# Zhongxu-Wang/ArtSpeech

Hardware: AMD Instinct MI355X
Metric: mel frames/sec (whole job; per-GPU = value / n_gpus), acoustic-model inference path, batch 32 x 200-frame utterances (higher is better)
Workload: dtype f32 (f16x3 split-operand MFMA, fp32 accumulate)

## Files before the change

### artspeech_amd/csrc/lstm.hip

```cpp
#include "common.h"
#include "artspeech_hip.h"
#define AS_FILE_CLS AS_CLS_LSTM

#define NB 2

static __device__ __forceinline__ float sigmoidf_(float x) { return __builtin_amdgcn_rcpf(1.0f + __expf(-x)); }
static __device__ __forceinline__ float tanhf_(float x)
{
    const float e = __expf(-2.0f * fabsf(x));
    const float t = (1.0f - e) * __builtin_amdgcn_rcpf(1.0f + e);
    return x < 0.f ? -t : t;
}

template <int CTRL>
static __device__ __forceinline__ float quad_dpp(float v)
{
    return __int_as_float(__builtin_amdgcn_mov_dpp(__float_as_int(v), CTRL, 0xf, 0xf, true));
}

struct LstmJobs { BiLstmJob j[AS_MAX_LSTM_JOBS]; };

static __device__ __forceinline__ void lds_barrier()
{
    asm volatile("s_waitcnt lgkmcnt(0)\n\ts_barrier" ::: "memory");
}

template <int HREG>
__global__ void __launch_bounds__(HREG ? 4 * HREG : 1024)
bilstm_kernel(const LstmJobs jobs, const int* __restrict__ col_off, int B, int Hrt)
{
    extern __shared__ __attribute__((aligned(16))) float sm[];
    const int H = HREG ? HREG : Hrt;
    float* hs = sm;
    float* gs = sm + 2 * H * NB;
    __shared__ int s_off[NB], s_len[NB];

    const BiLstmJob job = jobs.j[blockIdx.z];
    const int dir = blockIdx.y;
    const int u0 = blockIdx.x * NB;
    const int r = threadIdx.x;
    const int G = 4 * H;
    if (r < NB) {
        const int u = u0 + r;
        s_off[r] = u < B ? col_off[u] : 0;
        s_len[r] = u < B ? col_off[u + 1] - col_off[u] : 0;
    }
    for (int i = r; i < 2 * H * NB; i += G) hs[i] = 0.f;
    __syncthreads();
    int Lmax = 0;
#pragma unroll
    for (int u = 0; u < NB; ++u) Lmax = s_len[u] > Lmax ? s_len[u] : Lmax;

    const float* w = job.whh_t + (size_t)dir * H * G + r;
    float wreg[HREG ? HREG : 1];
    if (HREG) {
#pragma unroll
        for (int k = 0; k < HREG; ++k) wreg[k] = w[(size_t)k * G];
    }
    const int unit = r % H, q = r / H;
    float c = 0.f;

    auto load_gx = [&](int t, float (&g)[NB]) {
#pragma unroll
        for (int u = 0; u < NB; ++u) {
            const int L = s_len[u];
            const int pos = dir ? L - 1 - t : t;
            g[u] = (t < L) ? job.gx_tm[(size_t)(s_off[u] + pos) * job.ldg + dir * G + r] : 0.f;
        }
    };
    float gnext[NB];
    load_gx(0, gnext);

    for (int t = 0; t < Lmax; ++t) {
        const float* hc = hs + (t & 1) * H * NB;
        float* hn = hs + ((t + 1) & 1) * H * NB;
        float acc[NB];
#pragma unroll
        for (int u = 0; u < NB; ++u) acc[u] = gnext[u];
        if (t + 1 < Lmax) load_gx(t + 1, gnext);
        if (HREG) {
#pragma unroll
            for (int k = 0; k < HREG; ++k) {
                const float2 h2 = *reinterpret_cast<const float2*>(hc + k * NB);
                acc[0] += wreg[k] * h2.x; acc[1] += wreg[k] * h2.y;
            }
        } else {
            for (int k0 = 0; k0 < H; k0 += 8) {
                float wk[8];
#pragma unroll
                for (int i = 0; i < 8; ++i) wk[i] = w[(size_t)(k0 + i) * G];
#pragma unroll
                for (int i = 0; i < 8; ++i) {
                    const float2 h2 = *reinterpret_cast<const float2*>(hc + (k0 + i) * NB);
                    acc[0] += wk[i] * h2.x; acc[1] += wk[i] * h2.y;
                }
            }
        }
        *reinterpret_cast<float2*>(gs + r * NB) = make_float2(acc[0], acc[1]);
        lds_barrier();
        if (q < NB) {
            const int u = q;
            const int L = s_len[u];
            if (t < L) {
                const float ig = sigmoidf_(gs[(unit)*NB + u]);
                const float fg = sigmoidf_(gs[(H + unit) * NB + u]);
                const float gg = tanhf_(gs[(2 * H + unit) * NB + u]);
                const float og = sigmoidf_(gs[(3 * H + unit) * NB + u]);
                c = fg * c + ig * gg;
                const float hv = og * tanhf_(c);
                hn[unit * NB + u] = hv;
                const int pos = dir ? L - 1 - t : t;
                job.out[(size_t)(dir * H + unit) * job.ldo + s_off[u] + pos] = hv;
            }
        }
        lds_barrier();
    }
}

template <int H, int KREG, int KLDS>
__global__ void __launch_bounds__(2 * H)
bilstm_big_kernel(const LstmJobs jobs, const int* __restrict__ col_off, int B)
{
    constexpr int G = 4 * H, NT = 2 * H, KS = H - KREG - KLDS, SB = 4;
    static_assert(KS >= 0 && KS % SB == 0, "split of the k range");
    extern __shared__ __attribute__((aligned(16))) float sm[];
    float* hs = sm;
    float* gs = hs + 2 * H * NB;
    float* wl = gs + G * NB;
    __shared__ int s_off[NB], s_len[NB];

    const BiLstmJob job = jobs.j[blockIdx.z];
    const int dir = blockIdx.y;
    const int u0 = blockIdx.x * NB;
    const int tid = threadIdx.x;
    if (tid < NB) {
        const int u = u0 + tid;
        s_off[tid] = u < B ? col_off[u] : 0;
        s_len[tid] = u < B ? col_off[u + 1] - col_off[u] : 0;
    }
    for (int i = tid; i < 2 * H * NB; i += NT) hs[i] = 0.f;
    const float* w = job.whh_t + (size_t)dir * H * G + tid;
    float wa[KREG], wb[KREG];
#pragma unroll
    for (int k = 0; k < KREG; ++k) {
        wa[k] = w[(size_t)k * G];
        wb[k] = w[(size_t)k * G + NT];
    }
#pragma unroll 4
    for (int k = 0; k < KLDS; ++k) {
        wl[k * G + tid] = w[(size_t)(KREG + k) * G];
        wl[k * G + NT + tid] = w[(size_t)(KREG + k) * G + NT];
    }
    const float* ws = w + (size_t)(KREG + KLDS) * G;
    __syncthreads();
    int Lmax = 0;
#pragma unroll
    for (int u = 0; u < NB; ++u) Lmax = s_len[u] > Lmax ? s_len[u] : Lmax;
    const int unit = tid % H, q = tid / H;
    float c = 0.f;

    auto load_gx = [&](int t, float (&ga)[NB], float (&gb)[NB]) {
#pragma unroll
        for (int u = 0; u < NB; ++u) {
            const int L = s_len[u];
            const int pos = dir ? L - 1 - t : t;
            const float* p = job.gx_tm + (size_t)(s_off[u] + pos) * job.ldg + dir * G + tid;
            ga[u] = (t < L) ? p[0] : 0.f;
            gb[u] = (t < L) ? p[NT] : 0.f;
        }
    };
    float gna[NB], gnb[NB];
    load_gx(0, gna, gnb);

    for (int t = 0; t < Lmax; ++t) {
        asm volatile("" ::: "memory");
        const float* hc = hs + (t & 1) * H * NB;
        float* hn = hs + ((t + 1) & 1) * H * NB;
        float a0 = gna[0], a1 = gna[1], b0 = gnb[0], b1 = gnb[1];
        if (t + 1 < Lmax) load_gx(t + 1, gna, gnb);
        float ka[SB], kb[SB];
#pragma unroll
        for (int i = 0; i < SB; ++i) {
            ka[i] = ws[(size_t)i * G];
            kb[i] = ws[(size_t)i * G + NT];
        }
#pragma unroll
        for (int k = 0; k < KREG; ++k) {
            const float2 h2 = *reinterpret_cast<const float2*>(hc + k * NB);
            a0 += wa[k] * h2.x; a1 += wa[k] * h2.y;
            b0 += wb[k] * h2.x; b1 += wb[k] * h2.y;
            if ((k & 7) == 7) asm volatile("" ::: "memory");
        }
#pragma unroll 4
        for (int k = 0; k < KLDS; ++k) {
            const float va = wl[k * G + tid], vb = wl[k * G + NT + tid];
            const float2 h2 = *reinterpret_cast<const float2*>(hc + (KREG + k) * NB);
            a0 += va * h2.x; a1 += va * h2.y;
            b0 += vb * h2.x; b1 += vb * h2.y;
        }
        for (int k0 = 0; k0 < KS; k0 += SB) {
            float na[SB], nb[SB];
            const int kn = k0 + SB < KS ? k0 + SB : k0;
#pragma unroll
            for (int i = 0; i < SB; ++i) {
                na[i] = ws[(size_t)(kn + i) * G];
                nb[i] = ws[(size_t)(kn + i) * G + NT];
            }
#pragma unroll
            for (int i = 0; i < SB; ++i) {
                const float2 h2 = *reinterpret_cast<const float2*>(hc + (KREG + KLDS + k0 + i) * NB);
                a0 += ka[i] * h2.x; a1 += ka[i] * h2.y;
                b0 += kb[i] * h2.x; b1 += kb[i] * h2.y;
            }
#pragma unroll
            for (int i = 0; i < SB; ++i) { ka[i] = na[i]; kb[i] = nb[i]; }
        }
        *reinterpret_cast<float2*>(gs + tid * NB) = make_float2(a0, a1);
        *reinterpret_cast<float2*>(gs + (NT + tid) * NB) = make_float2(b0, b1);
        lds_barrier();
        {
            const int u = q;
            const int L = s_len[u];
            if (t < L) {
                const float ig = sigmoidf_(gs[(unit)*NB + u]);
                const float fg = sigmoidf_(gs[(H + unit) * NB + u]);
                const float gg = tanhf_(gs[(2 * H + unit) * NB + u]);
                const float og = sigmoidf_(gs[(3 * H + unit) * NB + u]);
                c = fg * c + ig * gg;
                const float hv = og * tanhf_(c);
                hn[unit * NB + u] = hv;
                const int pos = dir ? L - 1 - t : t;
                job.out[(size_t)(dir * H + unit) * job.ldo + s_off[u] + pos] = hv;
            }
        }
        lds_barrier();
    }
}

template <int H>
__global__ void __launch_bounds__(4 * H)
bilstm_quad_kernel(const LstmJobs jobs, const int* __restrict__ col_off, int B)
{
    constexpr int KQ = H / 4, G = 4 * H;
    __shared__ __attribute__((aligned(16))) float hs[2][H][NB];
    __shared__ int s_off[NB], s_len[NB];
    const BiLstmJob job = jobs.j[blockIdx.z];
    const int dir = blockIdx.y, u0 = blockIdx.x * NB;
    const int tid = threadIdx.x, unit = tid >> 2, kq = tid & 3;
    if (tid < NB) {
        const int u = u0 + tid;
        s_off[tid] = u < B ? col_off[u] : 0;
        s_len[tid] = u < B ? col_off[u + 1] - col_off[u] : 0;
    }
    for (int i = tid; i < 2 * H * NB; i += G) (&hs[0][0][0])[i] = 0.f;
    __syncthreads();
    const int L0 = s_len[0], L1 = s_len[1], o0 = s_off[0], o1 = s_off[1];
    const int Lmax = L0 > L1 ? L0 : L1;

    float w[4][KQ];
    const float* wp = job.whh_t + (size_t)dir * H * G + unit;
#pragma unroll
    for (int g = 0; g < 4; ++g)
#pragma unroll
        for (int kk = 0; kk < KQ; ++kk) w[g][kk] = wp[(size_t)(kq * KQ + kk) * G + g * H];

    const float* gxp = job.gx_tm + dir * G + kq * H + unit;
    auto load_gx = [&](int t, float& g0, float& g1) {
        g0 = (t < L0) ? gxp[(size_t)(o0 + (dir ? L0 - 1 - t : t)) * job.ldg] : 0.f;
        g1 = (t < L1) ? gxp[(size_t)(o1 + (dir ? L1 - 1 - t : t)) * job.ldg] : 0.f;
    };
    constexpr int PF = 4;
    float gq0[PF], gq1[PF];
#pragma unroll
    for (int j = 0; j < PF; ++j) load_gx(j, gq0[j], gq1[j]);
    float c = 0.f;
    const int my_u = kq & 1, my_L = my_u ? L1 : L0, my_o = my_u ? o1 : o0;

    for (int t0 = 0; t0 < Lmax; t0 += PF) {
#pragma unroll
      for (int j = 0; j < PF; ++j) {
        const int t = t0 + j;
        if (t >= Lmax) break;
        const float(*hc)[NB] = hs[t & 1];
        float(*hn)[NB] = hs[(t + 1) & 1];
        float acc[4][2];
#pragma unroll
        for (int g = 0; g < 4; ++g) {
            acc[g][0] = (g == kq) ? gq0[j] : 0.f;
            acc[g][1] = (g == kq) ? gq1[j] : 0.f;
        }
        load_gx(t + PF, gq0[j], gq1[j]);
#pragma unroll
        for (int kk = 0; kk < KQ; ++kk) {
            const float2 h2 = *reinterpret_cast<const float2*>(&hc[kq * KQ + kk][0]);
#pragma unroll
            for (int g = 0; g < 4; ++g) {
                acc[g][0] += w[g][kk] * h2.x;
                acc[g][1] += w[g][kk] * h2.y;
            }
        }
        float pre[4];
#pragma unroll
        for (int g = 0; g < 4; ++g) {
            float a0 = acc[g][0], a1 = acc[g][1];
            a0 += __shfl_xor(a0, 1); a1 += __shfl_xor(a1, 1);
            a0 += __shfl_xor(a0, 2); a1 += __shfl_xor(a1, 2);
            pre[g] = my_u ? a1 : a0;
        }
        if (kq < 2 && t < my_L) {
            const float ig = sigmoidf_(pre[0]), fg = sigmoidf_(pre[1]), gg = tanhf_(pre[2]), og = sigmoidf_(pre[3]);
            c = fg * c + ig * gg;
            const float hv = og * tanhf_(c);
            hn[unit][my_u] = hv;
            job.out[(size_t)(dir * H + unit) * job.ldo + my_o + (dir ? my_L - 1 - t : t)] = hv;
        }
        lds_barrier();
      }
    }
}

typedef float lf2 __attribute__((ext_vector_type(2)));
template <int H>
__global__ void __launch_bounds__(4 * H)
bilstm_quad1_kernel(const LstmJobs jobs, const int* __restrict__ col_off, int B)
{
    constexpr int KQ = H / 4, G = 4 * H;
    static_assert(KQ % 4 == 0, "quarter of the hidden vector in float4 steps");
    __shared__ __attribute__((aligned(16))) float hs[2][H];
    const BiLstmJob job = jobs.j[blockIdx.z];
    const int dir = blockIdx.y, u = blockIdx.x;
    const int tid = threadIdx.x, unit = tid >> 2, kq = tid & 3;
    const int o0 = col_off[u], L = col_off[u + 1] - o0;
    if (L <= 0) return;
    for (int i = tid; i < 2 * H; i += G) (&hs[0][0])[i] = 0.f;
    __syncthreads();

    lf2 wif[KQ], wgo[KQ];
    const float* wp = job.whh_t + (size_t)dir * H * G + unit;
#pragma unroll
    for (int kk = 0; kk < KQ; ++kk) {
        const float* r = wp + (size_t)(kq * KQ + kk) * G;
        wif[kk] = lf2{r[0], r[H]};
        wgo[kk] = lf2{r[2 * H], r[3 * H]};
    }
    const float* gxp = job.gx_tm + dir * G + kq * H + unit;
    auto load_gx = [&](int t) { return (t < L) ? gxp[(size_t)(o0 + (dir ? L - 1 - t : t)) * job.ldg] : 0.f; };
    constexpr int PF = 4;
    float gq[PF];
#pragma unroll
    for (int j = 0; j < PF; ++j) gq[j] = load_gx(j);
    float c = 0.f;
    float* outp = job.out + (size_t)(dir * H + unit) * job.ldo + o0;

    for (int t0 = 0; t0 < L; t0 += PF) {
#pragma unroll
        for (int j = 0; j < PF; ++j) {
            const int t = t0 + j;
            if (t >= L) break;
            const float* hc = hs[t & 1] + kq * KQ;
            float* hn = hs[(t + 1) & 1];
            const float gx = gq[j];
            gq[j] = load_gx(t + PF);
            lf2 aif0 = {0.f, 0.f}, ago0 = {0.f, 0.f}, aif1 = {0.f, 0.f}, ago1 = {0.f, 0.f};
#pragma unroll
            for (int k4 = 0; k4 < KQ; k4 += 4) {
                const float4 h4 = *reinterpret_cast<const float4*>(hc + k4);
                aif0 += wif[k4] * lf2{h4.x, h4.x};
                ago0 += wgo[k4] * lf2{h4.x, h4.x};
                aif1 += wif[k4 + 1] * lf2{h4.y, h4.y};
                ago1 += wgo[k4 + 1] * lf2{h4.y, h4.y};
                aif0 += wif[k4 + 2] * lf2{h4.z, h4.z};
                ago0 += wgo[k4 + 2] * lf2{h4.z, h4.z};
                aif1 += wif[k4 + 3] * lf2{h4.w, h4.w};
                ago1 += wgo[k4 + 3] * lf2{h4.w, h4.w};
            }
            float pre[4] = {aif0[0] + aif1[0], aif0[1] + aif1[1], ago0[0] + ago1[0], ago0[1] + ago1[1]};
#pragma unroll
            for (int g = 0; g < 4; ++g) {
                pre[g] += quad_dpp<0xB1>(pre[g]);
                pre[g] += quad_dpp<0x4E>(pre[g]);
            }
            const float sc = kq == 2 ? 2.f : 1.f;
            const float x = (kq == 0 ? pre[0] : kq == 1 ? pre[1] : kq == 2 ? pre[2] : pre[3]) + gx;
            const float act = fmaf(__builtin_amdgcn_rcpf(1.0f + __expf(-sc * x)), sc, 1.0f - sc);
            const float ig = quad_dpp<0x00>(act), fg = quad_dpp<0x55>(act), gg = quad_dpp<0xAA>(act), og = quad_dpp<0xFF>(act);
            c = fg * c + ig * gg;
            const float hv = og * fmaf(__builtin_amdgcn_rcpf(1.0f + __expf(-2.0f * c)), 2.0f, -1.0f);
            if (kq == 0) {
                hn[unit] = hv;
                outp[dir ? L - 1 - t : t] = hv;
            }
            lds_barrier();
        }
    }
}

extern "C" int as_bilstm_f32(const BiLstmJob* jobs_host, int n_jobs, const int32_t* col_off, int B, int H,
                             as_stream_t stream)
{
    if (!jobs_host || n_jobs <= 0 || n_jobs > AS_MAX_LSTM_JOBS || !col_off || B < 0 || H <= 0 || (4 * H) % 64 ||
        4 * H > 1024 || H % 8)
        return AS_EINVAL;
    LstmJobs jobs;
    for (int i = 0; i < AS_MAX_LSTM_JOBS; ++i) jobs.j[i] = jobs_host[i < n_jobs ? i : 0];
    for (int i = 0; i < n_jobs; ++i)
        if (!jobs.j[i].gx_tm || !jobs.j[i].whh_t || !jobs.j[i].out || jobs.j[i].ldg < 8 * H) return AS_EINVAL;
    if (B == 0) return AS_OK;
    const size_t smem = sizeof(float) * ((size_t)2 * H * NB + (size_t)4 * H * NB);
    const dim3 grid(as_cdiv(B, NB), 2, n_jobs), block(4 * H);
    AsProfScope prof__(AS_FILE_CLS, 0, 0, (hipStream_t)stream);
    const bool single = (H == 64 || H == 128) && (long)n_jobs * 2 * B <= 512;
    if (single) {
        const dim3 g1(B, 2, n_jobs);
        if (H == 64) hipLaunchKernelGGL(bilstm_quad1_kernel<64>, g1, block, 0, (hipStream_t)stream, jobs, col_off, B);
        else hipLaunchKernelGGL(bilstm_quad1_kernel<128>, g1, block, 0, (hipStream_t)stream, jobs, col_off, B);
        AS_CHECK_LAUNCH();
        return AS_OK;
    }
    switch (H) {
    case 16: hipLaunchKernelGGL(bilstm_quad_kernel<16>, grid, block, 0, (hipStream_t)stream, jobs, col_off, B); break;
    case 32: hipLaunchKernelGGL(bilstm_quad_kernel<32>, grid, block, 0, (hipStream_t)stream, jobs, col_off, B); break;
    case 64: hipLaunchKernelGGL(bilstm_quad_kernel<64>, grid, block, 0, (hipStream_t)stream, jobs, col_off, B); break;
    case 128: hipLaunchKernelGGL(bilstm_quad_kernel<128>, grid, block, 0, (hipStream_t)stream, jobs, col_off, B); break;
    case 256: {
        constexpr int KREG = 32, KLDS = 36;
        const size_t sm_big = smem + sizeof(float) * (size_t)KLDS * 1024;
        AS_LDS_OPT_IN((bilstm_big_kernel<256, KREG, KLDS>), (int)sm_big);
        hipLaunchKernelGGL((bilstm_big_kernel<256, KREG, KLDS>), grid, dim3(512), sm_big, (hipStream_t)stream, jobs, col_off, B);
        break;
    }
    default: hipLaunchKernelGGL(bilstm_kernel<0>, grid, block, smem, (hipStream_t)stream, jobs, col_off, B, H); break;
    }
    AS_CHECK_LAUNCH();
    return AS_OK;
}

#define CL_P 4
#define CL_REGION_WORDS 1032
static __device__ __forceinline__ float dpp_add8(float v)
{
    int x = __builtin_bit_cast(int, v);
    v += __builtin_bit_cast(float, __builtin_amdgcn_update_dpp(0, x, 0xB1, 0xF, 0xF, true));
    x = __builtin_bit_cast(int, v);
    v += __builtin_bit_cast(float, __builtin_amdgcn_update_dpp(0, x, 0x4E, 0xF, 0xF, true));
    x = __builtin_bit_cast(int, v);
    v += __builtin_bit_cast(float, __builtin_amdgcn_update_dpp(0, x, 0x141, 0xF, 0xF, true));
    return v;
}

template <int NBU>
__global__ void __launch_bounds__(512)
bilstm_cluster_kernel(const LstmJobs jobs, const int* __restrict__ col_off, int B, int n_clusters, unsigned long long* __restrict__ xchg,
                      unsigned* __restrict__ status, int spin_limit, int drop_member)
{
    constexpr int H = 256, G = 4 * H, UW = H / CL_P, KS = 8, KQ = H / KS, SL = KQ * NBU + 4, HB = KS * SL;
    __shared__ __attribute__((aligned(16))) float hs[2 * HB];
    const int lin = blockIdx.x;
    const int cl = (lin & 7) + 8 * ((lin >> 3) / CL_P), member = (lin >> 3) % CL_P;
    if (cl >= n_clusters) return;
    const int groups = (B + NBU - 1) / NBU;
    const int ug = cl % groups, dir = (cl / groups) & 1;
    const BiLstmJob job = jobs.j[cl / (2 * groups)];
    const int tid = threadIdx.x, ul = tid >> 3, kq = tid & 7, unit = member * UW + ul;
    int off[NBU], len[NBU], Lmax = 0;
#pragma unroll
    for (int i = 0; i < NBU; ++i) {
        const int u = ug * NBU + i;
        off[i] = u < B ? col_off[u] : 0;
        len[i] = u < B ? col_off[u + 1] - col_off[u] : 0;
        Lmax = len[i] > Lmax ? len[i] : Lmax;
    }
    if (Lmax <= 0) return;
    if (member == drop_member) return;
    unsigned long long* region = xchg + (size_t)cl * CL_REGION_WORDS;
    const unsigned epoch = (unsigned)region[0] & 0x7FFFu;
    const unsigned tagbase = epoch << 17;
    unsigned long long* words = region + 1;
    for (int i = tid; i < 2 * HB; i += 512) hs[i] = 0.f;

    lf2 wif[KQ], wgo[KQ];
    const float* wp = job.whh_t + (size_t)dir * H * G + unit;
#pragma unroll
    for (int kk = 0; kk < KQ; ++kk) {
        const float* r = wp + (size_t)(kq * KQ + kk) * G;
        wif[kk] = lf2{r[0], r[H]};
        wgo[kk] = lf2{r[2 * H], r[3 * H]};
    }
    const int gu = kq >> 2, gL = gu < NBU ? len[gu < NBU ? gu : 0] : 0, gO = off[gu < NBU ? gu : 0];
    const float* gxp = job.gx_tm + dir * G + (kq & 3) * H + unit;
    auto load_gx = [&](int t) { return (t < gL) ? gxp[(size_t)(gO + (dir ? gL - 1 - t : t)) * job.ldg] : 0.f; };
    constexpr int PF = 4;
    float gq[PF];
#pragma unroll
    for (int j = 0; j < PF; ++j) gq[j] = load_gx(j);
    float c = 0.f;
    const int my_u = kq < NBU ? kq : 0, my_L = len[my_u], my_o = off[my_u];
    float* outp = job.out + (size_t)(dir * H + unit) * job.ldo + my_o;
    const int pk = tid / NBU, pu = tid % NBU, ppos = (pk / KQ) * SL + (pk % KQ) * NBU + pu;
    __syncthreads();

    for (int t0 = 0; t0 < Lmax; t0 += PF) {
#pragma unroll
        for (int j = 0; j < PF; ++j) {
            const int t = t0 + j;
            if (t >= Lmax) break;
            float* hb = hs + (t & 1) * HB;
            if (t > 0 && tid < H * NBU) {
                const unsigned long long* w = words + (size_t)((t - 1) & 1) * H * NBU + tid;
                const unsigned want = tagbase | (unsigned)t;
                unsigned long long v = __hip_atomic_load(w, __ATOMIC_RELAXED, __HIP_MEMORY_SCOPE_AGENT);
                for (int spin = 0; (unsigned)(v >> 32) != want && spin < spin_limit; ++spin) {
                    __builtin_amdgcn_s_sleep(1);
                    v = __hip_atomic_load(w, __ATOMIC_RELAXED, __HIP_MEMORY_SCOPE_AGENT);
                }
                if ((unsigned)(v >> 32) != want) as_status_raise(status, AS_STATUS_LSTM_TIMEOUT);
                hb[ppos] = __uint_as_float((unsigned)v);
            }
            lds_barrier();
            const float gx = gq[j];
            gq[j] = load_gx(t + PF);
            lf2 aif[NBU], ago[NBU];
#pragma unroll
            for (int u = 0; u < NBU; ++u) {
                aif[u] = lf2{kq == 4 * u ? gx : 0.f, kq == 4 * u + 1 ? gx : 0.f};
                ago[u] = lf2{kq == 4 * u + 2 ? gx : 0.f, kq == 4 * u + 3 ? gx : 0.f};
            }
            const float* hc = hb + kq * SL;
            if (NBU == 2) {
#pragma unroll
                for (int kk = 0; kk < KQ; kk += 2) {
                    const float4 h4 = *reinterpret_cast<const float4*>(hc + kk * 2);
                    aif[0] += wif[kk] * lf2{h4.x, h4.x};
                    ago[0] += wgo[kk] * lf2{h4.x, h4.x};
                    aif[NBU - 1] += wif[kk] * lf2{h4.y, h4.y};
                    ago[NBU - 1] += wgo[kk] * lf2{h4.y, h4.y};
                    aif[0] += wif[kk + 1] * lf2{h4.z, h4.z};
                    ago[0] += wgo[kk + 1] * lf2{h4.z, h4.z};
                    aif[NBU - 1] += wif[kk + 1] * lf2{h4.w, h4.w};
                    ago[NBU - 1] += wgo[kk + 1] * lf2{h4.w, h4.w};
                }
            } else {
                lf2 bif = {0.f, 0.f}, bgo = {0.f, 0.f};
#pragma unroll
                for (int kk = 0; kk < KQ; kk += 4) {
                    const float4 h4 = *reinterpret_cast<const float4*>(hc + kk);
                    aif[0] += wif[kk] * lf2{h4.x, h4.x};
                    ago[0] += wgo[kk] * lf2{h4.x, h4.x};
                    bif += wif[kk + 1] * lf2{h4.y, h4.y};
                    bgo += wgo[kk + 1] * lf2{h4.y, h4.y};
                    aif[0] += wif[kk + 2] * lf2{h4.z, h4.z};
                    ago[0] += wgo[kk + 2] * lf2{h4.z, h4.z};
                    bif += wif[kk + 3] * lf2{h4.w, h4.w};
                    bgo += wgo[kk + 3] * lf2{h4.w, h4.w};
                }
                aif[0] += bif;
                ago[0] += bgo;
            }
            float pre[4] = {0.f, 0.f, 0.f, 0.f};
#pragma unroll
            for (int u = 0; u < NBU; ++u) {
                const float pi = dpp_add8(aif[u][0]), pf = dpp_add8(aif[u][1]), pg = dpp_add8(ago[u][0]), po = dpp_add8(ago[u][1]);
                if (u == my_u) { pre[0] = pi; pre[1] = pf; pre[2] = pg; pre[3] = po; }
            }
            if (kq < NBU) {
                float hv = 0.f;
                if (t < my_L) {
                    const float ig = sigmoidf_(pre[0]), fg = sigmoidf_(pre[1]), gg = tanhf_(pre[2]), og = sigmoidf_(pre[3]);
                    c = fg * c + ig * gg;
                    hv = og * tanhf_(c);
                    outp[dir ? my_L - 1 - t : t] = hv;
                }
                const unsigned long long word = ((unsigned long long)(tagbase | (unsigned)(t + 1)) << 32) | __float_as_uint(hv);
                __hip_atomic_store(words + (size_t)(t & 1) * H * NBU + unit * NBU + kq, word, __ATOMIC_RELAXED, __HIP_MEMORY_SCOPE_AGENT);
            }
        }
    }
    if (member == 0) {
        if (Lmax == 1 && tid < H * NBU) {
            const unsigned long long* w = words + tid;
            const unsigned want = tagbase | 1u;
            unsigned long long v = __hip_atomic_load(w, __ATOMIC_RELAXED, __HIP_MEMORY_SCOPE_AGENT);
            for (int spin = 0; (unsigned)(v >> 32) != want && spin < spin_limit; ++spin) {
                __builtin_amdgcn_s_sleep(1);
                v = __hip_atomic_load(w, __ATOMIC_RELAXED, __HIP_MEMORY_SCOPE_AGENT);
            }
            if ((unsigned)(v >> 32) != want) as_status_raise(status, AS_STATUS_LSTM_TIMEOUT);
        }
        __syncthreads();
        if (tid == 0) region[0] = epoch + 1;
    }
}

static int g_cl_drop_member = -1, g_cl_spin_limit = 1 << 21;
extern "C" int as_bilstm_cluster_test_hooks(int drop_member, int spin_limit)
{
    if (drop_member < -1 || drop_member >= CL_P || spin_limit < 0) return AS_EINVAL;
    g_cl_drop_member = drop_member;
    g_cl_spin_limit = spin_limit > 0 ? spin_limit : 1 << 21;
    return AS_OK;
}

extern "C" size_t as_bilstm_cluster_bytes(int n_jobs, int B)
{
    if (n_jobs <= 0 || B <= 0) return 0;
    return (size_t)n_jobs * 2 * B * CL_REGION_WORDS * sizeof(unsigned long long);
}

extern "C" int as_bilstm_cluster_f32(const BiLstmJob* jobs_host, int n_jobs, const int32_t* col_off, int B, int H, int max_len, void* xchg,
                                     size_t xchg_bytes, as_stream_t stream)
{
    if (!jobs_host || n_jobs <= 0 || n_jobs > AS_MAX_LSTM_JOBS || !col_off || B < 0 || H <= 0) return AS_EINVAL;
    if (B == 0) return AS_OK;
    const long c1 = (long)n_jobs * 2 * B, c2 = (long)n_jobs * 2 * ((B + 1) / 2);
    const int nbu = c1 * CL_P <= 256 ? 1 : (c2 * CL_P <= 256 ? 2 : 0);
    const char* mode = getenv("AS_LSTM_CLUSTER");
    const int use = mode ? atoi(mode) : nbu;
    if (H != 256 || !xchg || use <= 0 || use > 2 || max_len <= 0 || max_len >= (1 << 17) || (use == 1 ? c1 : c2) * CL_P > 256 ||
        xchg_bytes < as_bilstm_cluster_bytes(n_jobs, B))
        return as_bilstm_f32(jobs_host, n_jobs, col_off, B, H, stream);
    LstmJobs jobs;
    for (int i = 0; i < AS_MAX_LSTM_JOBS; ++i) jobs.j[i] = jobs_host[i < n_jobs ? i : 0];
    for (int i = 0; i < n_jobs; ++i)
        if (!jobs.j[i].gx_tm || !jobs.j[i].whh_t || !jobs.j[i].out || jobs.j[i].ldg < 8 * H) return AS_EINVAL;
    const int ncl = (int)(use == 1 ? c1 : c2);
    const dim3 grid(8 * CL_P * as_cdiv(ncl, 8)), block(512);
    unsigned* status = as_status_words_device();
    AsProfScope prof__(AS_FILE_CLS, 0, 0, (hipStream_t)stream);
    if (use == 1)
        hipLaunchKernelGGL(bilstm_cluster_kernel<1>, grid, block, 0, (hipStream_t)stream, jobs, col_off, B, ncl,
                           static_cast<unsigned long long*>(xchg), status, g_cl_spin_limit, g_cl_drop_member);
    else
        hipLaunchKernelGGL(bilstm_cluster_kernel<2>, grid, block, 0, (hipStream_t)stream, jobs, col_off, B, ncl,
                           static_cast<unsigned long long*>(xchg), status, g_cl_spin_limit, g_cl_drop_member);
    AS_CHECK_LAUNCH();
    return AS_OK;
}
```

Measured before the change: 1.806 million.

## Add MFMA BiLSTM kernel batching 16 utterances per workgroup for H=128

Adds a BiLSTM recurrence kernel for H=128 that processes 16 utterances per workgroup. The recurrent matmul runs on f16 MFMA instructions using a hi/lo split of both the scaled weights and the hidden state, accumulating in fp32. It keeps weights in registers, double-buffers the hidden state in LDS, prefetches the gate inputs and writes outputs in 4-step chunks. Dispatch moves into a rule header that selects this kernel when B>=16. The aim is to replace the per-utterance scalar quad-DPP recurrence with matrix-core work shared across utterances, at the cost of three MFMAs per product and some precision risk from the f16 split.

```diff
diff --git a/artspeech_amd/csrc/lstm.hip b/artspeech_amd/csrc/lstm.hip
--- a/artspeech_amd/csrc/lstm.hip
+++ b/artspeech_amd/csrc/lstm.hip
@@ -1,5 +1,6 @@
 #include "common.h"
 #include "artspeech_hip.h"
+#include "lstm_rule.h"
 #define AS_FILE_CLS AS_CLS_LSTM
 
 #define NB 2
@@ -395,6 +396,154 @@
     }
 }
 
+typedef _Float16 lh8 __attribute__((ext_vector_type(8)));
+typedef _Float16 lh4 __attribute__((ext_vector_type(4)));
+typedef float lf4 __attribute__((ext_vector_type(4)));
+typedef float lf4u __attribute__((ext_vector_type(4), aligned(4)));
+
+static __device__ __forceinline__ float rcp1p_exp2(float x) { return __builtin_amdgcn_rcpf(1.0f + __builtin_amdgcn_exp2f(x)); }
+
+__global__ void __launch_bounds__(512)
+bilstm_mfma_kernel(const LstmJobs jobs, const int* __restrict__ col_off, int B)
+{
+    constexpr int H = 128, G = 4 * H, KS = H / 32, NU = 16, PF = 2, ST = 4;
+    constexpr float L2E = 1.44269504088896341f, HSCALE = 4096.f;
+    static_assert(PF == 2 && ST % 2 == 0, "the step parity is the unrolled step's index, and a set of gate terms per parity");
+    __shared__ __attribute__((aligned(16))) _Float16 hb[2][2][KS][64][8];
+    __shared__ unsigned s_max[8];
+    const BiLstmJob job = jobs.j[blockIdx.z];
+    const int dir = blockIdx.y, u0 = blockIdx.x * NU;
+    const int tid = threadIdx.x, w = tid >> 6, lane = tid & 63, q = lane >> 4, n = lane & 15;
+
+    int Lmax = 0, L = 0, off = 0;
+    for (int i = 0; i < NU; ++i) {
+        const int u = u0 + i;
+        const int o = u < B ? col_off[u] : 0;
+        int len = u < B ? col_off[u + 1] - o : 0;
+        len = len > 0 ? len : 0;
+        Lmax = len > Lmax ? len : Lmax;
+        if (i == n) { L = len; off = o; }
+    }
+    if (Lmax == 0) return;
+
+    const float* wp = job.whh_t + (size_t)dir * H * G + 16 * w + n + (size_t)(8 * q) * G;
+    unsigned mx = 0;
+#pragma unroll
+    for (int ks = 0; ks < KS; ++ks)
+#pragma unroll
+        for (int j = 0; j < 8; ++j)
+#pragma unroll
+            for (int g = 0; g < 4; ++g) {
+                const unsigned a = __float_as_uint(wp[(size_t)(32 * ks + j) * G + g * H]) & 0x7FFFFFFFu;
+                mx = a > mx ? a : mx;
+            }
+#pragma unroll
+    for (int o = 32; o; o >>= 1) {
+        const unsigned other = (unsigned)__shfl_xor((int)mx, o);
+        mx = other > mx ? other : mx;
+    }
+    if (lane == 0) s_max[w] = mx;
+    const int slot = 16 * (2 * (w & 1) + (q >> 1)) + n, sj = 4 * (q & 1), sk = w >> 1;
+    *reinterpret_cast<lh4*>(&hb[0][0][sk][slot][sj]) = lh4{0, 0, 0, 0};
+    *reinterpret_cast<lh4*>(&hb[0][1][sk][slot][sj]) = lh4{0, 0, 0, 0};
+    __syncthreads();
+#pragma unroll
+    for (int i = 0; i < 8; ++i) mx = s_max[i] > mx ? s_max[i] : mx;
+    int E = (int)(mx >> 23);
+    E = E < 30 ? 30 : (E > 254 ? 254 : E);
+    const float wscale = __uint_as_float((unsigned)(267 - E) << 23);
+    const float undo = __uint_as_float((unsigned)(E - 25) << 23);
+
+    lh8 wh[4][KS], wl[4][KS];
+#pragma unroll
+    for (int ks = 0; ks < KS; ++ks)
+#pragma unroll
+        for (int j = 0; j < 8; ++j)
+#pragma unroll
+            for (int g = 0; g < 4; ++g) {
+                const float v = wp[(size_t)(32 * ks + j) * G + g * H] * wscale;
+                const _Float16 a = (_Float16)v;
+                wh[g][ks][j] = a;
+                wl[g][ks][j] = (_Float16)(v - (float)a);
+            }
+
+    const long gstride = dir ? -(long)job.ldg : (long)job.ldg;
+    const float* gp = job.gx_tm + dir * G + 16 * w + 4 * q + (size_t)(L > 0 ? off + (dir ? L - 1 : 0) : 0) * job.ldg;
+    auto load_gx = [&](lf4 (&g)[4]) {
+#pragma unroll
+        for (int gg = 0; gg < 4; ++gg) g[gg] = *reinterpret_cast<const lf4*>(gp + gg * H);
+    };
+    lf4 gq[PF][4];
+    load_gx(gq[0]);
+    gp += 1 < L ? gstride : 0;
+    float* outp = job.out + (size_t)(dir * H + 16 * w + 4 * q) * job.ldo + off;
+    float c[4] = {0.f, 0.f, 0.f, 0.f};
+    lh4 hh = {0, 0, 0, 0}, hl = {0, 0, 0, 0};
+
+    lf4 hq[4];
+    for (int t0 = 0; t0 < Lmax; t0 += ST) {
+#pragma unroll
+        for (int j = 0; j < ST; ++j) {
+            const int t = t0 + j;
+            if (t >= Lmax) break;
+            const int cur = j & 1;
+            load_gx(gq[cur ^ 1]);
+            __builtin_amdgcn_sched_barrier(0);
+            gp += t + 2 < L ? gstride : 0;
+            lf4 acc[4];
+#pragma unroll
+            for (int g = 0; g < 4; ++g) acc[g] = lf4{0.f, 0.f, 0.f, 0.f};
+#pragma unroll
+            for (int ks = 0; ks < KS; ++ks) {
+                const lh8 bh = *reinterpret_cast<const lh8*>(&hb[cur][0][ks][lane][0]);
+                const lh8 bl = *reinterpret_cast<const lh8*>(&hb[cur][1][ks][lane][0]);
+#pragma unroll
+                for (int g = 0; g < 4; ++g) acc[g] = __builtin_amdgcn_mfma_f32_16x16x32_f16(wh[g][ks], bl, acc[g], 0, 0, 0);
+#pragma unroll
+                for (int g = 0; g < 4; ++g) acc[g] = __builtin_amdgcn_mfma_f32_16x16x32_f16(wl[g][ks], bh, acc[g], 0, 0, 0);
+#pragma unroll
+                for (int g = 0; g < 4; ++g) acc[g] = __builtin_amdgcn_mfma_f32_16x16x32_f16(wh[g][ks], bh, acc[g], 0, 0, 0);
+            }
+            const lf4 (&gx)[4] = gq[cur];
+            const bool live = t < L;
+            float hv[4];
+#pragma unroll
+            for (int r = 0; r < 4; ++r) {
+                const float ig = rcp1p_exp2(-L2E * fmaf(acc[0][r], undo, gx[0][r]));
+                const float fg = rcp1p_exp2(-L2E * fmaf(acc[1][r], undo, gx[1][r]));
+                const float gg = fmaf(rcp1p_exp2(-2.f * L2E * fmaf(acc[2][r], undo, gx[2][r])), 2.f, -1.f);
+                const float og = rcp1p_exp2(-L2E * fmaf(acc[3][r], undo, gx[3][r]));
+                const float cn = fg * c[r] + ig * gg;
+                hv[r] = og * fmaf(rcp1p_exp2(-2.f * L2E * cn), 2.f, -1.f);
+                const float hs = hv[r] * HSCALE;
+                const _Float16 a = (_Float16)hs, b = (_Float16)(hs - (float)a);
+                c[r] = live ? cn : c[r];
+                hh[r] = live ? a : hh[r];
+                hl[r] = live ? b : hl[r];
+            }
+#pragma unroll
+            for (int r = 0; r < 4; ++r) hq[r][dir ? ST - 1 - j : j] = hv[r];
+            *reinterpret_cast<lh4*>(&hb[cur ^ 1][0][sk][slot][sj]) = hh;
+            *reinterpret_cast<lh4*>(&hb[cur ^ 1][1][sk][slot][sj]) = hl;
+            lds_barrier();
+        }
+        const int nl = L - t0;
+        if (nl >= ST) {
+            const int pos = dir ? L - t0 - ST : t0;
+#pragma unroll
+            for (int r = 0; r < 4; ++r) *reinterpret_cast<lf4u*>(outp + (size_t)r * job.ldo + pos) = hq[r];
+        } else if (nl > 0) {
+#pragma unroll
+            for (int j = 0; j < ST - 1; ++j)
+                if (j < nl) {
+                    const int pos = dir ? L - 1 - t0 - j : t0 + j;
+#pragma unroll
+                    for (int r = 0; r < 4; ++r) outp[(size_t)r * job.ldo + pos] = hq[r][dir ? ST - 1 - j : j];
+                }
+        }
+    }
+}
+
 extern "C" int as_bilstm_f32(const BiLstmJob* jobs_host, int n_jobs, const int32_t* col_off, int B, int H,
                              as_stream_t stream)
 {
@@ -406,27 +555,32 @@
     for (int i = 0; i < n_jobs; ++i)
         if (!jobs.j[i].gx_tm || !jobs.j[i].whh_t || !jobs.j[i].out || jobs.j[i].ldg < 8 * H) return AS_EINVAL;
     if (B == 0) return AS_OK;
+    const lstm_rule::Rule rl = lstm_rule::rule(H, B, n_jobs);
     const size_t smem = sizeof(float) * ((size_t)2 * H * NB + (size_t)4 * H * NB);
-    const dim3 grid(as_cdiv(B, NB), 2, n_jobs), block(4 * H);
+    const dim3 grid(rl.gx, rl.gy, rl.gz), block(rl.threads);
+    if (rl.form == lstm_rule::MFMA)
+        for (int i = 0; i < n_jobs; ++i)
+            if (jobs.j[i].ldg % 4 || (uintptr_t)jobs.j[i].gx_tm % 16) return AS_EINVAL;
     AsProfScope prof__(AS_FILE_CLS, 0, 0, (hipStream_t)stream);
-    const bool single = (H == 64 || H == 128) && (long)n_jobs * 2 * B <= 512;
-    if (single) {
-        const dim3 g1(B, 2, n_jobs);
-        if (H == 64) hipLaunchKernelGGL(bilstm_quad1_kernel<64>, g1, block, 0, (hipStream_t)stream, jobs, col_off, B);
-        else hipLaunchKernelGGL(bilstm_quad1_kernel<128>, g1, block, 0, (hipStream_t)stream, jobs, col_off, B);
-        AS_CHECK_LAUNCH();
-        return AS_OK;
-    }
-    switch (H) {
-    case 16: hipLaunchKernelGGL(bilstm_quad_kernel<16>, grid, block, 0, (hipStream_t)stream, jobs, col_off, B); break;
-    case 32: hipLaunchKernelGGL(bilstm_quad_kernel<32>, grid, block, 0, (hipStream_t)stream, jobs, col_off, B); break;
-    case 64: hipLaunchKernelGGL(bilstm_quad_kernel<64>, grid, block, 0, (hipStream_t)stream, jobs, col_off, B); break;
-    case 128: hipLaunchKernelGGL(bilstm_quad_kernel<128>, grid, block, 0, (hipStream_t)stream, jobs, col_off, B); break;
-    case 256: {
+    switch (rl.form) {
+    case lstm_rule::MFMA: hipLaunchKernelGGL(bilstm_mfma_kernel, grid, block, 0, (hipStream_t)stream, jobs, col_off, B); break;
+    case lstm_rule::SINGLE:
+        if (H == 64) hipLaunchKernelGGL(bilstm_quad1_kernel<64>, grid, block, 0, (hipStream_t)stream, jobs, col_off, B);
+        else hipLaunchKernelGGL(bilstm_quad1_kernel<128>, grid, block, 0, (hipStream_t)stream, jobs, col_off, B);
+        break;
+    case lstm_rule::PAIR:
+        switch (H) {
+        case 16: hipLaunchKernelGGL(bilstm_quad_kernel<16>, grid, block, 0, (hipStream_t)stream, jobs, col_off, B); break;
+        case 32: hipLaunchKernelGGL(bilstm_quad_kernel<32>, grid, block, 0, (hipStream_t)stream, jobs, col_off, B); break;
+        case 64: hipLaunchKernelGGL(bilstm_quad_kernel<64>, grid, block, 0, (hipStream_t)stream, jobs, col_off, B); break;
+        default: hipLaunchKernelGGL(bilstm_quad_kernel<128>, grid, block, 0, (hipStream_t)stream, jobs, col_off, B); break;
+        }
+        break;
+    case lstm_rule::BIG: {
         constexpr int KREG = 32, KLDS = 36;
         const size_t sm_big = smem + sizeof(float) * (size_t)KLDS * 1024;
         AS_LDS_OPT_IN((bilstm_big_kernel<256, KREG, KLDS>), (int)sm_big);
-        hipLaunchKernelGGL((bilstm_big_kernel<256, KREG, KLDS>), grid, dim3(512), sm_big, (hipStream_t)stream, jobs, col_off, B);
+        hipLaunchKernelGGL((bilstm_big_kernel<256, KREG, KLDS>), grid, block, sm_big, (hipStream_t)stream, jobs, col_off, B);
         break;
     }
     default: hipLaunchKernelGGL(bilstm_kernel<0>, grid, block, smem, (hipStream_t)stream, jobs, col_off, B, H); break;
diff --git a/artspeech_amd/csrc/lstm_rule.h b/artspeech_amd/csrc/lstm_rule.h
--- /dev/null
+++ b/artspeech_amd/csrc/lstm_rule.h
@@ -0,0 +1,32 @@
+#pragma once
+#include <cstdint>
+
+namespace lstm_rule {
+
+enum Form : int32_t { STREAM = 0, PAIR = 1, SINGLE = 2, BIG = 3, MFMA = 4 };
+
+constexpr int MFMA_UTTS = 16;
+constexpr int MFMA_MIN_B = 16;
+constexpr int SINGLE_MAX_WG = 512;
+
+struct Rule {
+    int32_t form, utts;
+    int32_t gx, gy, gz;
+    int32_t threads;
+};
+
+inline Rule rule(int H, int B, int n_jobs)
+{
+    Rule r;
+    if (H == 128 && B >= MFMA_MIN_B) { r.form = MFMA; r.utts = MFMA_UTTS; r.threads = 512; }
+    else if ((H == 64 || H == 128) && (long)n_jobs * 2 * B <= SINGLE_MAX_WG) { r.form = SINGLE; r.utts = 1; r.threads = 4 * H; }
+    else if (H == 16 || H == 32 || H == 64 || H == 128) { r.form = PAIR; r.utts = 2; r.threads = 4 * H; }
+    else if (H == 256) { r.form = BIG; r.utts = 2; r.threads = 512; }
+    else { r.form = STREAM; r.utts = 2; r.threads = 4 * H; }
+    r.gx = B > 0 ? (B + r.utts - 1) / r.utts : 0;
+    r.gy = 2;
+    r.gz = n_jobs;
+    return r;
+}
+
+}
```

After: 1.805 million. About the same (-0.0%).
